# dcmlr/groundgrid

Measured on NVIDIA H100. Metric: Mpoints/sec segmented (64-beam scan), higher is better.
Workload: dtype f32/f64

## Files before the change

### groundgrid_b200/csrc/gg_capi.cu

```cuda
#include <cuda.h>
#include <cuda_runtime.h>

#include <cmath>
#include <cstdarg>
#include <cstdio>
#include <atomic>
#include <chrono>
#include <condition_variable>
#include <cstdlib>
#include <cstring>
#include <functional>
#include <initializer_list>
#include <mutex>
#include <string>
#include <thread>
#include <vector>

#include "gg_host.h"
#include "gg_internal.h"

namespace {

thread_local std::string g_last_error;

// ... 745 lines not shown
        v.visits = d_vs;
        v.levels = (int)ls.size() - 1;
        h->sched_levels = v.levels;
        h->sched_visits = (int)vs.size();
        for (size_t l = 0; l + 1 < ls.size(); ++l) h->sched_max = std::max(h->sched_max, ls[l + 1] - ls[l]);
        v.spiral_recs = nullptr;
        v.spiral_dist = 0;
        v.spiral_threads = h->sched_max <= 512 ? 512 : 1024;
        int dist = 2;
        if (const char* e = getenv("GG_SPIRAL_DIST")) dist = atoi(e);
        std::vector<uint32_t> rc;
        int max_recent = 0;
        if (dist >= 1 && dist <= 3 && h->sched_max <= 1024 && gg::build_spiral_records(n, v.k.res_sq, ls, vs, dist, rc, max_recent)) {
            uint32_t* d_rc = nullptr;
            GG_TRY(dev_alloc(h, &d_rc, rc.size() + 4));
            GG_CUDA_TRY(cudaMemcpy(d_rc, rc.data(), rc.size() * sizeof(uint32_t), cudaMemcpyHostToDevice));
            v.spiral_recs = reinterpret_cast<const uint4*>(d_rc);
            v.spiral_dist = dist;
        }
        std::memset(&v.skew, 0, sizeof(v.skew));
        int want_skew = 1;
        if (const char* e = getenv("GG_SPIRAL_SKEW")) want_skew = atoi(e);
        gg::SkewTables sk;
        if (want_skew) gg::build_spiral_skew(n, ls, vs, sk);
        int M = 32, phases = 1, M_thr = 32, phases_thr = 1;
        if (sk.ok) {
            const int kGap = 2 * 8 + 4;
            auto smallest_fitting = [&](int m0) {
                int m = m0;
                for (; m < sk.KP; m += 32) {
                    bool fits = true;
                    for (int sd = 0; sd < 4 && fits; ++sd)
                        for (int c0 = 0; c0 + m < sk.KP && fits; ++c0) {
                            const int a = sd * sk.KP + c0, b2 = a + m;
                            if (sk.lane_begin[a] < sk.lane_end[a] && sk.lane_begin[b2] < sk.lane_end[b2] &&
                                sk.lane_end[a] + kGap > sk.lane_begin[b2])
                                fits = false;
                        }
                    if (fits) break;
                }
                return std::min(m, sk.KP);
            };
            M = (4 * sk.KP + 64 <= 1024) ? sk.KP : smallest_fitting(32);
            phases = (sk.KP + M - 1) / M;
            int m0 = 0;
            if (const char* e = getenv("GG_SPIRAL_M")) m0 = atoi(e) / 32 * 32;
            M_thr = m0 <= 0 ? M : smallest_fitting(std::max(32, m0));
// ... 2 lines not shown
        }
        if (sk.ok) {
            const int irr_max = std::max(1, sk.max_irr_per_level);
            const int irr_words = ((irr_max * 22 + 3) / 4) * 4;
            std::vector<uint32_t> blocks((size_t)(sk.levels + 4) * irr_words, 0xffffffffu);
            for (int l = 0; l < sk.levels; ++l)
                for (int r = sk.irr_level_start[l]; r < sk.irr_level_start[l + 1]; ++r) {
                    const uint32_t* w = &sk.irr_recs[(size_t)r * 16];
                    const int vv = r - sk.irr_level_start[l];
                    uint32_t* blk = &blocks[(size_t)l * irr_words];
                    for (int q = 0; q < 9; ++q) {
                        blk[(vv * 9 + q) * 2] = w[1 + q];
                        blk[(vv * 9 + q) * 2 + 1] = 0xffffffffu;
                    }
                    const uint32_t ents[4] = {w[10] & 0xffffu, w[10] >> 16, w[11] & 0xffffu, w[11] >> 16};
                    for (uint32_t e : ents)
                        if (e != 0xffffu) blk[(vv * 9 + (e >> 12)) * 2 + 1] = e & 4095u;
                    uint32_t* hd = blk + irr_max * 18 + vv * 4;
                    hd[0] = w[0];
                    hd[1] = w[12];
                    hd[2] = w[13];
                    hd[3] = w[14];
                }
            auto upload_phases = [&](int m_, int phases_, const int** d_b, const int** d_e, const int** d_c) -> int {
                std::vector<int> ph_b((size_t)phases_ * 4 * m_, 0), ph_e((size_t)phases_ * 4 * m_, 0), ph_c((size_t)phases_ * 4 * m_, 0);
                for (int ph = 0; ph < phases_; ++ph)
                    for (int sd = 0; sd < 4; ++sd)
                        for (int m = 0; m < m_; ++m) {
                            const int col = ph * m_ + m;
                            if (col >= sk.KP) continue;
                            const size_t dst = ((size_t)ph * 4 + sd) * m_ + m;
                            ph_b[dst] = sk.lane_begin[sd * sk.KP + col];
                            ph_e[dst] = sk.lane_end[sd * sk.KP + col];
                            ph_c[dst] = sk.lane_cell0[sd * sk.KP + col];
                        }
                int *d_lb = nullptr, *d_le = nullptr, *d_lc = nullptr;
                int rc2;
                if ((rc2 = dev_alloc(h, &d_lb, ph_b.size())) || (rc2 = dev_alloc(h, &d_le, ph_e.size())) || (rc2 = dev_alloc(h, &d_lc, ph_c.size())))
                    return rc2;
                if (cudaMemcpy(d_lb, ph_b.data(), ph_b.size() * sizeof(int), cudaMemcpyHostToDevice) != cudaSuccess ||
                    cudaMemcpy(d_le, ph_e.data(), ph_e.size() * sizeof(int), cudaMemcpyHostToDevice) != cudaSuccess ||
                    cudaMemcpy(d_lc, ph_c.data(), ph_c.size() * sizeof(int), cudaMemcpyHostToDevice) != cudaSuccess)
                    return fail(GG_E_CUDA, "upload of the spiral phase tables failed");
                *d_b = d_lb;
                *d_e = d_le;
                *d_c = d_lc;
// ... 24 lines not shown
            int want_async = 0;
            if (const char* e = getenv("GG_SPIRAL_ASYNC")) want_async = atoi(e);
            auto upload_req = [&](int m_, const uint16_t** d_req) -> int {
                *d_req = nullptr;
                std::vector<uint16_t> rq;
                int n_agents = 0;
                if (!want_async || !gg::build_skew_sync(sk, m_, gg::SKEW_XCH_ASYNC, rq, n_agents)) return GG_OK;
                uint16_t* d = nullptr;
                int rc2;
                if ((rc2 = dev_alloc(h, &d, rq.size()))) return rc2;
                if (cudaMemcpy(d, rq.data(), rq.size() * sizeof(uint16_t), cudaMemcpyHostToDevice) != cudaSuccess)
                    return fail(GG_E_CUDA, "upload of the spiral synchronisation table failed");
                *d_req = d;
                return GG_OK;
            };
            v.skew.sync_sleep = 20;
            if (const char* e = getenv("GG_SPIRAL_SLEEP")) v.skew.sync_sleep = std::max(0, atoi(e));
            GG_TRY(upload_req(M, &v.skew.req));
            if (M_thr == M)
                v.skew.thr_req = v.skew.req;
            else
                GG_TRY(upload_req(M_thr, &v.skew.thr_req));
            v.skew.irr_blocks = reinterpret_cast<const uint4*>(d_irr);
            v.skew.irr_max = irr_max;
            v.skew.irr_chunks = irr_words / 4;
            v.skew.KP = sk.KP;
            v.skew.rows = sk.rows;
            v.skew.row0 = sk.row0;
            v.skew.lanes = sk.lanes;
            v.skew.levels = sk.levels;
            std::memcpy(v.skew.pattern, sk.pattern, sizeof(sk.pattern));
        }
    }

    if (const char* e = getenv("GG_LAUNCH_UNIT")) h->launch_unit = std::max(1, atoi(e));
    if (const char* e = getenv("GG_COPY_STREAMS")) h->n_copy_in = std::min(8, std::max(1, atoi(e)));
    if (const char* e = getenv("GG_MAIN_HELP")) h->main_help = atoi(e);
    if (const char* e = getenv("GG_RAW_GATE")) h->raw_gate = std::max(1, atoi(e));
    if (const char* e = getenv("GG_BUS_TARGET_MB")) h->bus_target = (size_t)std::max(0, atoi(e)) << 20;
    if (const char* e = getenv("GG_RAW_DEPTH")) h->raw_depth = std::min(8, std::max(1, atoi(e)));
    if (const char* e = getenv("GG_HOST_PACK")) {
        h->host_pack = atoi(e) ? 1 : 0;
        h->host_pack_mix = 0;
    }
    v.packed = nullptr;
    if (stream) {
// ... 1186 lines not shown
```

### groundgrid_b200/csrc/gg_host.cpp

```cpp
#include <immintrin.h>

#include <algorithm>
#include <cmath>
#include <cstdio>
#include <thread>
#include <cstdint>
#include <cpuid.h>
#include <cstdlib>
#include <cstring>
#include <vector>

#include <sched.h>

#include "gg_host.h"

namespace gg {

int cells_per_side(double dimension_m, float resolution) {
    return (int)std::round((float)dimension_m / resolution);
}

void build_expected_points(int n, std::vector<float>& table) {
    const float vertical_point_ang_dist = 0.00174532925 * 2;
    table.assign((size_t)n * n, 0.0f);
// ... 169 lines not shown
        }
        if (nr > 4) ok = false;
        max_recent = std::max(max_recent, nr);
        const float fx = (float)x - (float)c, fy = (float)y - (float)c;
        const bool far = ((double)fx * (double)fx + (double)fy * (double)fy) * res_sq > 12.0;
        recs[4 * (size_t)t + 0] = (uint32_t)x | ((uint32_t)y << 16);
        recs[4 * (size_t)t + 1] = r[0] | (r[1] << 16);
        recs[4 * (size_t)t + 2] = r[2] | (r[3] << 16);
        recs[4 * (size_t)t + 3] = (far ? 1u : 0u) | (seen[cell] ? 2u : 0u);
        last_writer[cell] = t;
        ++seen[cell];
    };
    for (int p = c - 1; p >= 1; --p) {
        const int side = (c - p) * 2;
        const int q = p + side;
        for (int pos = p; pos < q; ++pos) visit(p, pos);
        for (int pos = p; pos < q; ++pos) visit(pos, p);
        for (int pos = q; pos >= p; --pos) visit(q, pos);
        for (int pos = q; pos >= p; --pos) visit(pos, q);
    }
    return ok;
}

void build_spiral_skew(int n, const std::vector<int>& level_start, const std::vector<uint32_t>& visits, SkewTables& t) {
    t = SkewTables();
    t.n = n;
    const int c = n / 2 - 1;
    const int K = c - 1;
    t.K = K;
    t.levels = (int)level_start.size() - 1;
    if (K < 2) return;
    t.KP = ((K + 2 + 31) / 32) * 32;
    if (4 * t.KP > 4095) return;
    const size_t nv = visits.size();
    std::vector<std::vector<int>> cell_levels((size_t)n * n);
    for (int l = 0; l < t.levels; ++l)
        for (int v = level_start[l]; v < level_start[l + 1]; ++v) {
            const int x = visits[v] & 0xffff, y = visits[v] >> 16;
            cell_levels[x + (size_t)y * n].push_back(l);
        }
    struct Visit {
        int s, k, j, x, y, level;
    };
    std::vector<Visit> seq;
    seq.reserve(nv);
    std::vector<int> seen((size_t)n * n, 0);
    int max_level = 0;
    auto push = [&](int s, int k, int j, int x, int y) {
        const size_t cell = x + (size_t)y * n;
// ... 61 lines not shown
            const int* h = homes(v.x - 1 + q % 3, v.y - 1 + q / 3);
            for (int i = 0; i < 4 && h[i] >= 0; ++i) bump(v.s * 9 + q, h[i] - own);
        }
    }
    for (int i = 0; i < 36; ++i) {
        int best = 0, cnt = -1;
        for (auto& e : stat[i])
            if (e.second > cnt) {
                cnt = e.second;
                best = e.first;
            }
        if (cnt < 0) return;
        t.pattern[i] = best;
    }

    std::vector<int> last_level((size_t)n * n, -1000000), last_lane((size_t)n * n, -1);
    t.lane_begin.assign(t.lanes, 0);
    t.lane_end.assign(t.lanes, 0);
    t.lane_cell0.assign(t.lanes, 0);
    std::vector<int> reg_first(t.lanes, -1), reg_last(t.lanes, -1), reg_count(t.lanes, 0);
    struct Irr {
        int level;
        uint32_t w[16];
    };
    std::vector<Irr> irr;
    for (const Visit& v : seq) {
        const int lane = v.s * t.KP + (v.k + 1);
        const int own = slot(v.s, v.k, v.level);
        const size_t cell = v.x + (size_t)v.y * n;
        int nb[9];
        bool regular = true;
        uint32_t rec[4] = {0xffffu, 0xffffu, 0xffffu, 0xffffu};
        int nrec = 0;
        for (int q = 0; q < 9; ++q) {
            const int cx = v.x - 1 + q % 3, cy = v.y - 1 + q / 3;
            const int* h = homes(cx, cy);
            if (h[0] < 0) return;
            const int want = own + t.pattern[v.s * 9 + q];
            bool match = false;
            for (int i = 0; i < 4 && h[i] >= 0; ++i) match |= (h[i] == want);
            nb[q] = match ? want : h[0];
            if (!match) regular = false;
            const size_t ncell = cx + (size_t)cy * n;
            const int back = v.level - last_level[ncell];
            if (back < 1) return;
            if (back == 1) {
                if (!(q == t.prev_q[v.s] && last_lane[ncell] == lane)) regular = false;
                if (nrec < 4) rec[nrec] = ((uint32_t)q << 12) | (uint32_t)last_lane[ncell];
                ++nrec;
            }
        }
        if (nrec > 4) return;
        if (nrec != 1) regular = false;
        const int* hown = homes(v.x, v.y);
        int mirror = -1;
        if (hown[1] >= 0) {
            regular = false;
            mirror = (hown[0] == own) ? hown[1] : hown[0];
            if (hown[2] >= 0) return;
        }
        {
            SkewTables::Access a;
            a.level = v.level;
            a.lane = lane;
            a.own = own;
            a.mirror = mirror;
            a.cell = (int)cell;
            a.regular = regular;
            for (int q = 0; q < 9; ++q) {
                a.nb[q] = nb[q];
                a.recent_lane[q] = -1;
            }
            for (int e = 0; e < 4; ++e)
                if (rec[e] != 0xffffu) a.recent_lane[rec[e] >> 12] = (int)(rec[e] & 4095u);
            t.acc.push_back(a);
        }
        if (regular) {
            ++t.n_regular;
            if (reg_first[lane] < 0) {
                reg_first[lane] = v.level;
                t.lane_cell0[lane] = (int)cell;
            }
            if (reg_last[lane] >= 0 && v.level != reg_last[lane] + 1) return;
            reg_last[lane] = v.level;
            ++reg_count[lane];
        } else {
            ++t.n_irregular;
            Irr r;
            r.level = v.level;
            std::memset(r.w, 0, sizeof(r.w));
            r.w[0] = (uint32_t)own;
            for (int q = 0; q < 9; ++q) r.w[1 + q] = (uint32_t)nb[q];
            r.w[10] = rec[0] | (rec[1] << 16);
            r.w[11] = rec[2] | (rec[3] << 16);
            r.w[12] = (uint32_t)mirror;
            r.w[13] = (uint32_t)lane;
            r.w[14] = (uint32_t)cell;
            irr.push_back(r);
        }
        last_level[cell] = v.level;
        last_lane[cell] = lane;
    }
    for (int l = 0; l < t.lanes; ++l)
        if (reg_first[l] >= 0) {
            t.lane_begin[l] = reg_first[l];
            t.lane_end[l] = reg_last[l] + 1;
            if (t.lane_end[l] - t.lane_begin[l] != reg_count[l]) return;
        }
    t.irr_level_start.assign((size_t)t.levels + 1, 0);
    for (const Irr& r : irr) ++t.irr_level_start[(size_t)r.level + 1];
    for (int l = 0; l < t.levels; ++l) {
        t.max_irr_per_level = std::max(t.max_irr_per_level, t.irr_level_start[(size_t)l + 1]);
        t.irr_level_start[(size_t)l + 1] += t.irr_level_start[l];
    }
    if (t.max_irr_per_level > 32) return;
    t.irr_recs.assign(irr.size() * 16, 0u);
    std::vector<int> cur(t.irr_level_start.begin(), t.irr_level_start.end() - 1);
    for (const Irr& r : irr) std::memcpy(&t.irr_recs[(size_t)cur[r.level]++ * 16], r.w, sizeof(r.w));
    t.ok = true;
}

bool build_skew_sync(const SkewTables& t, int M, int xch_depth, std::vector<uint16_t>& req, int& n_agents) {
    req.clear();
    n_agents = 0;
    if (!t.ok || M < 32 || (M % 32) != 0 || xch_depth < 2 || (xch_depth & (xch_depth - 1))) return false;
    const int lane_agents = 4 * M / 32;
    if (lane_agents + 1 > 32 || t.levels >= 65535) return false;
    n_agents = lane_agents + 1;
    const int IRR = lane_agents, L = t.levels;
    req.assign((size_t)n_agents * L * 32, 0);
    bool ok = true;
    auto agent_of = [&](const SkewTables::Access& a) {
        if (!a.regular) return IRR;
        const int side = a.lane / t.KP, col = a.lane % t.KP;
        return (side * M + col % M) / 32;
    };
    auto need = [&](int a, int lvl, int b, int done) {
        if (a == b || b < 0) return;
        if (lvl < 0) lvl = 0;
        if (done + 1 > lvl) {
            if (getenv("GG_SYNC_DEBUG")) fprintf(stderr, "sync: agent %d level %d needs agent %d done %d\n", a, lvl, b, done);
// ... 274 lines not shown
    if (ok && req && req_cap >= (int)r.size()) std::memcpy(req, r.data(), r.size() * sizeof(uint16_t));
    return ok ? 1 : 0;
}

int gg_host_spiral_skew(int n, int* header, int* pattern, int* lane_begin, int* lane_end, int* cell_home, int* irr_level_start,
                        uint32_t* irr_recs, int irr_cap_words) {
    std::vector<int> ls;
    std::vector<uint32_t> vs;
    gg::build_spiral_schedule(n, ls, vs);
    gg::SkewTables t;
    gg::build_spiral_skew(n, ls, vs, t);
    const int h[10] = {t.ok ? 1 : 0, t.K, t.KP, t.rows, t.levels, t.row0, t.lanes, (int)t.n_irregular, t.max_irr_per_level, (int)t.n_regular};
    std::memcpy(header, h, sizeof(h));
    if (!t.ok) return 0;
    if (pattern) std::memcpy(pattern, t.pattern, sizeof(t.pattern));
    if (lane_begin) std::memcpy(lane_begin, t.lane_begin.data(), t.lane_begin.size() * sizeof(int));
    if (lane_end) std::memcpy(lane_end, t.lane_end.data(), t.lane_end.size() * sizeof(int));
    if (cell_home) std::memcpy(cell_home, t.cell_home.data(), t.cell_home.size() * sizeof(int));
    if (irr_level_start) std::memcpy(irr_level_start, t.irr_level_start.data(), t.irr_level_start.size() * sizeof(int));
    if (irr_recs && irr_cap_words >= (int)t.irr_recs.size()) std::memcpy(irr_recs, t.irr_recs.data(), t.irr_recs.size() * sizeof(uint32_t));
    return 1;
}

int gg_host_move_map(double res, double* pos_xy, double nx, double ny, int* shift_ij) {
    gg::move_map(res, pos_xy[0], pos_xy[1], nx, ny, shift_ij[0], shift_ij[1]);
    return (shift_ij[0] != 0 || shift_ij[1] != 0) ? 1 : 0;
}

int gg_host_geometry_constants(double dimension_m, float resolution, unsigned flags, double* out) {
    gg::Const k;
    gg::derive_geometry(dimension_m, resolution, flags, k);
    const double v[9] = {(double)k.N, (double)k.N2, (double)k.full_layers, (double)k.res_f, k.res, k.rres, k.len, k.half, k.res_sq};
    std::memcpy(out, v, sizeof(v));
    return 0;
}

int gg_host_config_constants(const gg_config* cfg, double* out) {
    gg::CfgConst k;
    gg::derive_config(*cfg, k);
    const double v[16] = {(double)k.max_ring, (double)k.pc_var_thresh_f, k.min_outlier_conf, k.outlier_tol, k.gp_thresh, k.df_sq, k.mdf_sq,
                          k.mdf10_sq, k.psc_sq, k.occ_factor, k.occ_factor2, k.dec_factor, k.lab_fac, k.lab_thres, k.lab_obs,
                          (double)k.decay_floor_ok};
    std::memcpy(out, v, sizeof(v));
    return 0;
}

// ... 32 lines not shown
```

### groundgrid_b200/csrc/gg_host.h

```cpp
#pragma once
#include <cstdint>
#include <vector>

#include "gg_internal.h"

namespace gg {
int cells_per_side(double dimension_m, float resolution);
void build_expected_points(int n, std::vector<float>& table);
void derive_geometry(double dimension_m, float resolution, unsigned flags, Const& k);
void derive_config(const gg_config& c, CfgConst& k);

class ConfigRegistry {
  public:
    void reset(int n_slots, const CfgConst& k);
    int assign(int slot, const CfgConst& k, bool* build);
    void invalidate(int id) { vars_[id].k.reserved = 1; }
    int variant_of(int slot) const { return slot_var_[slot]; }
    const CfgConst& constants(int id) const { return vars_[id].k; }
    int refs(int id) const { return vars_[id].refs; }
    int live() const;
    int ids() const { return (int)vars_.size(); }

  private:
    struct Variant {
// ... 2 lines not shown
    };
    std::vector<Variant> vars_;
    std::vector<int> slot_var_;
};
void move_map(double res, double& px, double& py, double nx, double ny, int& shift_i, int& shift_j);
void build_spiral_schedule(int n, std::vector<int>& level_start, std::vector<uint32_t>& visits);
void pack_cloud_range(const gg_point* src, size_t n, unsigned char* dst, size_t i0, size_t i1, bool cached = false);
int usable_cpus();

struct SkewTables {
    bool ok = false;
    int n = 0, K = 0, KP = 0, rows = 0, levels = 0, row0 = 8;
    int lanes = 0;
    size_t slots = 0;
    int pattern[36] = {0};
    int prev_q[4] = {1, 3, 7, 5};
    std::vector<int> lane_begin, lane_end;
    std::vector<int> lane_cell0;
    std::vector<int> cell_home;
    std::vector<int> irr_level_start;
    std::vector<uint32_t> irr_recs;
    int max_irr_per_level = 0;
    size_t n_regular = 0, n_irregular = 0;
    struct Access {
        int level, lane;
        int own, mirror, cell;
        int nb[9];
        int recent_lane[9];
        bool regular;
    };
    std::vector<Access> acc;
};
bool build_skew_sync(const SkewTables& t, int M, int xch_depth, std::vector<uint16_t>& req, int& n_agents);
void build_spiral_skew(int n, const std::vector<int>& level_start, const std::vector<uint32_t>& visits, SkewTables& t);
bool build_spiral_records(int n, double res_sq, const std::vector<int>& level_start, const std::vector<uint32_t>& visits,
                          int dist, std::vector<uint32_t>& recs, int& max_recent);
}

extern "C" {
int gg_host_cells_per_side(double dimension_m, float resolution);
int gg_host_expected_points(double dimension_m, float resolution, float* dst);
int gg_host_spiral_schedule(int n, int* level_start, int level_cap, uint32_t* visits, int visit_cap, int* n_levels, int* n_visits);
int gg_host_spiral_records(int n, float resolution, int dist, uint32_t* recs, int rec_cap_words, int* max_recent);
int gg_host_move_map(double res, double* pos_xy, double nx, double ny, int* shift_ij);
int gg_host_geometry_constants(double dimension_m, float resolution, unsigned flags, double* out);
int gg_host_config_constants(const gg_config* cfg, double* out);
int gg_host_config_registry(int n_slots, int n_ops, const int* op_slot, const gg_config* op_cfg, int* out);
int gg_host_pack_cloud(const gg_point* src, size_t n, unsigned char* dst);
int gg_host_pack_cloud_cached(const gg_point* src, size_t n, unsigned char* dst);
int gg_host_packer_selftest(int threads, int n_jobs, size_t n_points, int ring_slots, int rounds, int lag);
int gg_host_spiral_skew_sync(int n, int M, int xch_depth, uint16_t* req, int req_cap, int* n_agents);
int gg_host_spiral_skew(int n, int* header, int* pattern, int* lane_begin, int* lane_end, int* cell_home, int* irr_level_start, uint32_t* irr_recs, int irr_cap_words);
}
```

### groundgrid_b200/csrc/gg_internal.h

```cpp
#pragma once
#include <cuda.h>
#include <cuda_runtime.h>
#include <stdint.h>

#include "groundgrid_b200.h"

namespace gg {

enum Layer : int {
    L_GROUND = 0,
    L_GROUNDPATCH = 1,
    L_OBSTACLES = 2,
    L_VARIANCE = 3,
    L_MINH = 4,
    L_COUNT = 5,
    L_MAXH = 6,
    L_GCAND = 7,
    L_PLANEDIST = 8,
    L_M2 = 9,
    L_MEAN = 10,
    L_RAW = 11,
    L_NUM = 12,
    L_NUM_LIVE = 6,
};
// ... 34 lines not shown
    CfgConst cfg;
    const float4* detect_tab;
    double px, py;
    double t20, t21, t22, t23;
    float ox, oy, oz;
    float base_z_f;
    int n_points;
    int shift_i, shift_j;
    int slot;
    const gg_point* src;
    const float* packed;
};

struct OutDest {
    uint8_t* labels;
    uint32_t* index;
    gg_point* cloud;
    int* count;
    unsigned select;
    int reserved;
};

constexpr int SKEW_XCH_ASYNC = 4;
struct SkewView {
    float2* sk;
    float* sd;
    size_t slots;
    const int* cell_home;
    const int* ph_begin;
    const int* ph_end;
    const int* ph_cell0;
    int M, phases;
    const int* thr_ph_begin;
    const int* thr_ph_end;
    const int* thr_ph_cell0;
    int thr_M, thr_phases;
    const uint16_t* req;
    const uint16_t* thr_req;
    int sync_sleep;
    const uint4* irr_blocks;
    int irr_max, irr_chunks;
    int KP, rows, row0, lanes, levels;
    int pattern[36];
};

struct View {
    Const k;
    float* layers;
    int n_layers;
    const float* expected;
    gg_point* points;
    unsigned char* packed;
    uint2* zw;
    uint32_t* runj;
    float* zsorted;
    uint2* rundir;
    float* dist;
    uint32_t* code;
    uint8_t* labels;
    unsigned long long* cnt64;
    int* raw_i;
    int* cellstart;
    int4* worklist;
    int* wl_count;
    int* cell_agg;
    int cell_tiles;
// ... 68 lines not shown
```

### groundgrid_b200/csrc/gg_kernels.cu

```cuda
#include <cuda.h>

#include <cfloat>
#include <cstddef>
#include <cstdio>

#include "gg_internal.h"

namespace gg {
constexpr int GRID_STRIDE_BLOCKS = 132;

__device__ __forceinline__ int trunc_index(double v) {
    if (!(v == v)) return 1000000000;
    if (v > 1.0e9) return 1000000000;
    if (v < -1.0e9) return -1000000000;
    return __double2int_rz(v);
}

__device__ __forceinline__ int trunc_quotient(double a, double res, double rres) {
    const double q = __dmul_rn(a, rres);
    const double f = __dsub_rn(q, rint(q));
    if (fabs(q) < 1.0e6 && fabs(f) > 1.0e-6) return __double2int_rz(q);
    return trunc_index(__ddiv_rn(a, res));
}

// ... 1225 lines not shown
}

constexpr int SKEW_IRR_THREADS = 64;
constexpr int SKEW_RING = 16;
constexpr int SKEW_STAGE_LEAD = 10;

__device__ __forceinline__ void prefetch_l2(const void* p) { asm volatile("prefetch.global.L2 [%0];" ::"l"(p)); }
__device__ __forceinline__ void prefetch_l1(const void* p) { asm volatile("prefetch.global.L1 [%0];" ::"l"(p)); }

__device__ __forceinline__ void skew_publish(int* s_prog, int agent, int completed, int lane) {
    __syncwarp();
    if (lane == 0) asm volatile("st.release.cta.shared.u32 [%0], %1;" ::"r"(smem_u32(s_prog + agent)), "r"(completed) : "memory");
}
__device__ __forceinline__ void skew_wait(const int* s_prog, int need, int lane, int sleep_ns) {
    const uint32_t addr = smem_u32(s_prog + lane);
    for (;;) {
        int p;
        asm volatile("ld.acquire.cta.shared.u32 %0, [%1];" : "=r"(p) : "r"(addr) : "memory");
        if (__all_sync(0xffffffffu, p >= need)) break;
        if (sleep_ns) __nanosleep(sleep_ns);
    }
}

template <int SIDE, bool ASYNC>
__device__ __forceinline__ void skew_lane_thread(const View& v, const SlotParams& sp, float2* s_xch, int* s_prog) {
    const SkewView& w = v.skew;
    constexpr int XM = (ASYNC ? SKEW_XCH_ASYNC : 2) - 1;
    const int lane_id = threadIdx.x & 31;
    const int agent = threadIdx.x >> 5;
    const uint16_t* __restrict__ req = ASYNC ? w.req + (size_t)agent * w.levels * 32 + lane_id : nullptr;
    int need_nxt = ASYNC ? (int)__ldg(req) : 0;
    constexpr int PQ = SIDE == 0 ? 1 : (SIDE == 1 ? 3 : (SIDE == 2 ? 7 : 5));
    constexpr int PF_FAR = 8, PF_NEAR = 2;
    const int L = w.levels, KP = w.KP, lanes = w.lanes, M = w.M;
    const int m = threadIdx.x - SIDE * M;
    float2* __restrict__ SK = w.sk + (size_t)sp.slot * w.slots;
    const float* __restrict__ SD = w.sd + (size_t)sp.slot * w.slots;
    float* __restrict__ Gn = v.layer(sp.slot, L_GROUND);
    float* __restrict__ Cn = v.layer(sp.slot, L_GROUNDPATCH);
    const int cstep = SIDE == 0 ? v.k.N : (SIDE == 1 ? 1 : (SIDE == 2 ? -v.k.N : -1));
    int off[9];
#pragma unroll
    for (int q = 0; q < 9; ++q) off[q] = w.pattern[SIDE * 9 + q];
    int off_new = off[0];
#pragma unroll
    for (int q = 1; q < 9; ++q) off_new = max(off_new, off[q]);

    int ph = -1, lb = 0, le = 0, base0 = 0, cell0 = 0, xid = 0;
    int w_first = 0, w_last = 0;
    auto next_phase = [&]() {
        ++ph;
        const size_t e = ((size_t)ph * 4 + SIDE) * M + m;
        const int col = ph * M + m;
        lb = w.ph_begin[e];
        le = w.ph_end[e];
        base0 = (SIDE * w.rows + w.row0) * KP + col;
        cell0 = w.ph_cell0[e] - lb * cstep;
        xid = SIDE * KP + col;
    };
    auto warp_window = [&]() {
        w_first = lb < le ? lb - PF_FAR : 0x7fffffff;
        w_last = lb < le ? le : -1;
#pragma unroll
        for (int d = 16; d >= 1; d >>= 1) {
            w_first = min(w_first, __shfl_xor_sync(0xffffffffu, w_first, d));
            w_last = max(w_last, __shfl_xor_sync(0xffffffffu, w_last, d));
        }
        w_first = max(w_first, 0) & ~1;
    };
    next_phase();
    warp_window();

    float2 A[9], B[9];
    float dA = -1.0f, dB = -1.0f;
#pragma unroll
    for (int q = 0; q < 9; ++q) A[q] = B[q] = make_float2(0.f, 0.f);
    if (lb == 0 && le > 0) {
#pragma unroll
        for (int q = 0; q < 9; ++q) A[q] = SK[base0 + off[q]];
        dA = SD[base0];
    }
#define GG_LANE_LEVEL(l_, CUR, CURD, NXT, NXTD)                                                      \
    {                                                                                               \
        const int l__ = (l_);                                                                       \
        if (ASYNC) {                                                                                \
            const int need__ = need_nxt;                                                            \
            if (l__ + 1 < L) need_nxt = (int)__ldg(req + (size_t)(l__ + 1) * 32);                   \
            skew_wait(s_prog, need__, lane_id, w.sync_sleep);                                                     \
        }                                                                                           \
        if (l__ + PF_FAR >= lb && l__ + PF_FAR < le) {                                              \
            prefetch_l2(SK + (base0 + (l__ + PF_FAR) * KP + off_new));                              \
            prefetch_l2(SD + (base0 + (l__ + PF_FAR) * KP));                                        \
        }                                                                                           \
        if (l__ + PF_NEAR >= lb && l__ + PF_NEAR < le) {                                            \
            prefetch_l1(SK + (base0 + (l__ + PF_NEAR) * KP + off_new));                             \
            prefetch_l1(SD + (base0 + (l__ + PF_NEAR) * KP));                                       \
        }                                                                                           \
        if (l__ + 1 >= lb && l__ + 1 < le) {                                                        \
            const float2* p__ = SK + (base0 + (l__ + 1) * KP);                                      \
            _Pragma("unroll") for (int q = 0; q < 9; ++q) NXT[q] = p__[off[q]];                    \
            NXTD = SD[base0 + (l__ + 1) * KP];                                                      \
        }                                                                                           \
        if (l__ >= lb && l__ < le) {                                                                \
            CUR[PQ] = s_xch[((l__ - 1) & XM) * lanes + xid];                                        \
            const float2 r__ = spiral_visit(CUR, CURD);                                             \
            s_xch[(l__ & XM) * lanes + xid] = r__;                                                  \
            SK[base0 + l__ * KP] = r__;                                                             \
            Gn[cell0 + l__ * cstep] = r__.x;                                                        \
            if (CURD >= 0.0f) Cn[cell0 + l__ * cstep] = r__.y;                                      \
        }                                                                                           \
        if (ASYNC)                                                                                  \
            skew_publish(s_prog, agent, l__ + 1, lane_id);                                          \
        else                                                                                        \
            __syncthreads();                                                                        \
    }
    for (int l = 0; l < L; l += 2) {
        if (w.phases > 1) {
            bool moved = false;
            while (ph + 1 < w.phases && l >= le) {
                next_phase();
                moved = true;
            }
            if (__any_sync(0xffffffffu, moved)) warp_window();
        }
        if (l < w_first || l >= w_last) {
            if (ASYNC) {
                skew_publish(s_prog, agent, min(l + 2, L), lane_id);
                if (l + 2 < L) need_nxt = (int)__ldg(req + (size_t)(l + 2) * 32);
            } else {
                __syncthreads();
                if (l + 1 < L) __syncthreads();
            }
            continue;
        }
        GG_LANE_LEVEL(l, A, dA, B, dB)
        if (l + 1 < L) GG_LANE_LEVEL(l + 1, B, dB, A, dA)
    }
#undef GG_LANE_LEVEL
}

__device__ __forceinline__ void skew_named_barrier() { asm volatile("bar.sync 1, %0;" ::"n"(SKEW_IRR_THREADS) : "memory"); }

template <bool ASYNC>
__device__ __forceinline__ void skew_irregular_thread(const View& v, const SlotParams& sp, float2* s_xch, uint4* s_ring, float2* s_nb, float* s_dd, int* s_prog) {
    const SkewView& w = v.skew;
    const int ti = threadIdx.x - 4 * w.M;
    constexpr int XM = (ASYNC ? SKEW_XCH_ASYNC : 2) - 1;
    const int lane_id = threadIdx.x & 31;
    const int agent = 4 * w.M / 32;
    const uint16_t* __restrict__ req = ASYNC ? w.req + (size_t)agent * w.levels * 32 + lane_id : nullptr;
    int need_nxt = ASYNC ? (int)__ldg(req) : 0;
    const int L = w.levels, lanes = w.lanes;
    const int chunks = w.irr_chunks, irr_max = w.irr_max;
    float2* __restrict__ SK = w.sk + (size_t)sp.slot * w.slots;
    const float* __restrict__ SD = w.sd + (size_t)sp.slot * w.slots;
    const uint4* __restrict__ blocks = w.irr_blocks;
    float* __restrict__ Gn = v.layer(sp.slot, L_GROUND);
    float* __restrict__ Cn = v.layer(sp.slot, L_GROUNDPATCH);
    if (ti == 0) {
        const int cidx = v.k.N / 2 - 1;
        Cn[cidx + cidx * v.k.N] = 1.0f;
        Gn[cidx + cidx * v.k.N] = sp.base_z_f;
    }
    const uint32_t* ring_w = reinterpret_cast<const uint32_t*>(s_ring);
    const int ring_words = chunks * 4;
    const bool stager = ti < chunks;
    const bool gatherer = ti < irr_max * 9;
    const bool visitor = ti < irr_max;

    if (stager) {
        for (int b = 0; b < SKEW_STAGE_LEAD; ++b) s_ring[b * chunks + ti] = blocks[(size_t)min(b, L + 3) * chunks + ti];
    }
    uint4 stage = stager ? blocks[(size_t)min(SKEW_STAGE_LEAD, L + 3) * chunks + ti] : make_uint4(0, 0, 0, 0);
    skew_named_barrier();
    float2 val = make_float2(0.f, 0.f);
    float dval = -1.0f;
    uint32_t info = 0xffffffffu;
    bool have = false;
    if (gatherer) {
        const uint32_t slot = ring_w[0 * ring_words + ti * 2], rl = ring_w[0 * ring_words + ti * 2 + 1];
        have = slot != 0xffffffffu;
        if (have) {
            val = SK[slot];
            info = rl;
            if (ti % 9 == 4) dval = SD[slot];
        }
    }
    for (int l = 0; l < L; ++l) {
        if (ASYNC) {
            const int need = need_nxt;
            if (l + 1 < L) need_nxt = (int)__ldg(req + (size_t)(l + 1) * 32);
            skew_wait(s_prog, need, lane_id, w.sync_sleep);
        }
        if (stager) {
            s_ring[((l + SKEW_STAGE_LEAD) % SKEW_RING) * chunks + ti] = stage;
            stage = blocks[(size_t)min(l + SKEW_STAGE_LEAD + 1, L + 3) * chunks + ti];
        }
        if (gatherer) {
            if (have) {
                if (info != 0xffffffffu) val = s_xch[((l - 1) & XM) * lanes + (int)info];
                s_nb[ti] = val;
                if (ti % 9 == 4) s_dd[ti / 9] = dval;
            }
            const uint32_t far_slot = ring_w[((l + SKEW_STAGE_LEAD - 2) % SKEW_RING) * ring_words + ti * 2];
            if (far_slot != 0xffffffffu) {
                prefetch_l2(SK + far_slot);
                if (ti % 9 == 4) prefetch_l2(SD + far_slot);
            }
            const uint32_t near_slot = ring_w[((l + 3) % SKEW_RING) * ring_words + ti * 2];
            if (near_slot != 0xffffffffu) {
                prefetch_l1(SK + near_slot);
                if (ti % 9 == 4) prefetch_l1(SD + near_slot);
            }
            const uint32_t* e = ring_w + ((l + 1) % SKEW_RING) * ring_words + ti * 2;
            const uint32_t slot = e[0];
            have = (l + 1 < L) && slot != 0xffffffffu;
            if (have) {
                val = SK[slot];
                info = e[1];
                if (ti % 9 == 4) dval = SD[slot];
            }
        }
        skew_named_barrier();
        if (visitor) {
            const uint32_t* hd = ring_w + (l % SKEW_RING) * ring_words + irr_max * 18 + ti * 4;
            const uint32_t own = hd[0];
            if (own != 0xffffffffu) {
                float2 nb[9];
#pragma unroll
                for (int q = 0; q < 9; ++q) nb[q] = s_nb[ti * 9 + q];
                const float2 r = spiral_visit(nb, s_dd[ti]);
                const int mirror = (int)hd[1];
                s_xch[(l & XM) * lanes + (int)hd[2]] = r;
                SK[own] = r;
                if (mirror >= 0) SK[mirror] = r;
                Gn[hd[3]] = r.x;
                if (s_dd[ti] >= 0.0f) Cn[hd[3]] = r.y;
            }
        }
        if (ASYNC) {
            skew_named_barrier();
            if (ti == 0) asm volatile("st.release.cta.shared.u32 [%0], %1;" ::"r"(smem_u32(s_prog + agent)), "r"(l + 1) : "memory");
        } else {
            __syncthreads();
        }
    }
}

template <int MAXT, int MIN_CTAS = 1, bool ASYNC = false>
__global__ void __launch_bounds__(MAXT, MIN_CTAS) k_spiral_skew(View v, const SlotParams* __restrict__ batch) {
    extern __shared__ __align__(16) unsigned char s_raw[];
    const SkewView& w = v.skew;
    uint4* s_ring = reinterpret_cast<uint4*>(s_raw);
    float2* s_xch = reinterpret_cast<float2*>(s_ring + SKEW_RING * w.irr_chunks);
    float2* s_nb = s_xch + (ASYNC ? SKEW_XCH_ASYNC : 2) * w.lanes;
    float* s_dd = reinterpret_cast<float*>(s_nb + w.irr_max * 9);
    int* s_prog = reinterpret_cast<int*>(s_dd + w.irr_max);
    const SlotParams& sp = batch[blockIdx.x];
    const int tid = threadIdx.x;
    if (ASYNC) {
        if (tid < 32) s_prog[tid] = tid <= 4 * w.M / 32 ? 0 : 0x7fffffff;
        __syncthreads();
    }
    if (tid < 4 * w.M) {
        const int side = tid / w.M;
        if (side == 0)
            skew_lane_thread<0, ASYNC>(v, sp, s_xch, s_prog);
        else if (side == 1)
            skew_lane_thread<1, ASYNC>(v, sp, s_xch, s_prog);
        else if (side == 2)
            skew_lane_thread<2, ASYNC>(v, sp, s_xch, s_prog);
        else
            skew_lane_thread<3, ASYNC>(v, sp, s_xch, s_prog);
    } else {
        skew_irregular_thread<ASYNC>(v, sp, s_xch, s_ring, s_nb, s_dd, s_prog);
    }
}

constexpr int LABEL_ILP = 4;

__global__ void __launch_bounds__(256) k_label(View v, const SlotParams* __restrict__ batch) {
    const SlotParams& sp = batch[blockIdx.y];
    const Const& k = v.k;
    const size_t base = (size_t)sp.slot * v.pcap;
    const int i0 = blockIdx.x * (256 * LABEL_ILP) + threadIdx.x;
    const int n = sp.n_points;
    if (i0 >= n) return;
    const float* L0 = v.layer(sp.slot, 0);
    const float* G = L0 + L_GROUND * k.N2;
    const float* V = L0 + L_VARIANCE * k.N2;
    float* OBS = v.layer(sp.slot, L_OBSTACLES);

    uint32_t code[LABEL_ILP];
    float dist[LABEL_ILP], z[LABEL_ILP], gh[LABEL_ILP], var[LABEL_ILP];
#pragma unroll
    for (int u = 0; u < LABEL_ILP; ++u) {
        const int i = i0 + u * 256;
        const bool in = i < n;
        code[u] = in ? v.code[base + i] : (PC_ABSENT << 24);
// ... 418 lines not shown
        else
            GG_LAUNCH(K_DETECT, k_detect_tma<4><<<tgrid, dim3(DT_X, DT_Y), 0, st>>>(v, batch, *layer_map));
    } else if (detect_occ >= 5)
        GG_LAUNCH(K_DETECT, k_detect_ldg<5><<<dgrid, dim3(DT_X, DT_Y), 0, st>>>(v, batch));
    else
        GG_LAUNCH(K_DETECT, k_detect_ldg<4><<<dgrid, dim3(DT_X, DT_Y), 0, st>>>(v, batch));
    ++launches;
    if (after_detect) cudaEventRecord(after_detect, st);
    if (stop_after == 2) return launches;

    if (v.skew.sk) {
        static const int share_min = getenv("GG_SPIRAL_SHARE_MIN") ? atoi(getenv("GG_SPIRAL_SHARE_MIN")) : 9;
        View vs = v;
        if (count >= share_min) {
            vs.skew.M = v.skew.thr_M;
            vs.skew.phases = v.skew.thr_phases;
            vs.skew.ph_begin = v.skew.thr_ph_begin;
            vs.skew.ph_end = v.skew.thr_ph_end;
            vs.skew.ph_cell0 = v.skew.thr_ph_cell0;
            vs.skew.req = v.skew.thr_req;
        }
        const bool async = vs.skew.req != nullptr;
        const int threads = 4 * vs.skew.M + SKEW_IRR_THREADS;
        const size_t shm = (size_t)SKEW_RING * v.skew.irr_chunks * sizeof(uint4) + (size_t)(async ? SKEW_XCH_ASYNC : 2) * v.skew.lanes * sizeof(float2) +
                           (size_t)v.skew.irr_max * 9 * sizeof(float2) + (size_t)v.skew.irr_max * sizeof(float) + 32 * sizeof(int) + 16;
#define GG_SKEW_LAUNCH(T, C)                                                                                                     \
    {                                                                                                                            \
        if (shm > 48 * 1024) {                                            \
            cudaFuncSetAttribute(k_spiral_skew<T, C, false>, cudaFuncAttributeMaxDynamicSharedMemorySize, (int)shm);             \
            cudaFuncSetAttribute(k_spiral_skew<T, C, true>, cudaFuncAttributeMaxDynamicSharedMemorySize, (int)shm);              \
        }                                                                                                                        \
        if (async)                                                                                                               \
            GG_LAUNCH(K_SPIRAL, (k_spiral_skew<T, C, true><<<count, threads, shm, st>>>(vs, batch)));                            \
        else                                                                                                                     \
            GG_LAUNCH(K_SPIRAL, (k_spiral_skew<T, C, false><<<count, threads, shm, st>>>(vs, batch)));                           \
    }
        if (threads <= 320)
            GG_SKEW_LAUNCH(320, 3)
        else if (threads <= 448)
            GG_SKEW_LAUNCH(448, 2)
        else if (threads <= 768)
            GG_SKEW_LAUNCH(768, 1)
        else
            GG_SKEW_LAUNCH(1024, 1)
#undef GG_SKEW_LAUNCH
    } else if (v.spiral_recs) {
        const size_t shm = (size_t)((v.levels + 4) & ~3) * sizeof(int) + (size_t)(v.spiral_dist + 1) * v.spiral_threads * sizeof(float2);
#define GG_SPIRAL_CASE(T, D)                                                                      \
    if (v.spiral_threads == T && v.spiral_dist == D) {                                            \
        if (shm > 48 * 1024) cudaFuncSetAttribute(k_spiral_pipe<T, D>, cudaFuncAttributeMaxDynamicSharedMemorySize, (int)shm); \
        GG_LAUNCH(K_SPIRAL, k_spiral_pipe<T, D><<<count, T, shm, st>>>(v, batch));                \
    }
        GG_SPIRAL_CASE(512, 1)
        GG_SPIRAL_CASE(512, 2)
        GG_SPIRAL_CASE(512, 3)
        GG_SPIRAL_CASE(1024, 1)
        GG_SPIRAL_CASE(1024, 2)
        GG_SPIRAL_CASE(1024, 3)
#undef GG_SPIRAL_CASE
    } else {
// ... 151 lines not shown
```

Before: 4940.

## Keep spiral neighbour values in a shared-memory level window instead of global copies

Adds a windowed variant of the skewed spiral kernel that keeps the last eight levels of results in shared memory and reads neighbour values from that ring instead of from global SK copies. The host checks that no lane overwrites a ring slot before its consumer reads it, and falls back to the old path otherwise. This removes global stores of mirror/own copies and their reloads. The cost is more shared memory per block, a 64-register cap, and extra host table building.

After: 5050 (median of 6 runs). 1.02x the previous value.

```diff
diff --git a/groundgrid_b200/csrc/gg_capi.cu b/groundgrid_b200/csrc/gg_capi.cu
--- a/groundgrid_b200/csrc/gg_capi.cu
+++ b/groundgrid_b200/csrc/gg_capi.cu
@@ -791,7 +791,18 @@
         int want_skew = 1;
         if (const char* e = getenv("GG_SPIRAL_SKEW")) want_skew = atoi(e);
         gg::SkewTables sk;
-        if (want_skew) gg::build_spiral_skew(n, ls, vs, sk);
+        int want_window = 1;
+        if (const char* e = getenv("GG_SPIRAL_WINDOW")) want_window = atoi(e);
+        if (want_skew) {
+            gg::build_spiral_skew(n, ls, vs, sk, want_window != 0);
+            if (sk.window) {
+                int smem_optin = 0;
+                cudaDeviceGetAttribute(&smem_optin, cudaDevAttrMaxSharedMemoryPerBlockOptin, h->device);
+                const size_t win_bytes = (size_t)gg::SKEW_WIN_ROWS * sk.lanes * sizeof(float2) + 16 * 1024;
+                if (!sk.ok || ((sk.win_bad >> (gg::SKEW_WIN_ROWS - 1)) & 1) || win_bytes > (size_t)smem_optin)
+                    gg::build_spiral_skew(n, ls, vs, sk);
+            }
+        }
         int M = 32, phases = 1, M_thr = 32, phases_thr = 1;
         if (sk.ok) {
             const int kGap = 2 * 8 + 4;
@@ -840,6 +851,18 @@
                     hd[2] = w[13];
                     hd[3] = w[14];
                 }
+            std::vector<uint32_t> win_blocks;
+            if (sk.window) {
+                win_blocks = blocks;
+                for (int l = 0; l < sk.levels; ++l)
+                    for (int r = sk.irr_level_start[l]; r < sk.irr_level_start[l + 1]; ++r)
+                        for (int q = 0; q < 9; ++q) {
+                            const uint32_t e = sk.irr_win[(size_t)r * 9 + q];
+                            const int row = (l - (int)(e >> 16)) & (gg::SKEW_WIN_ROWS - 1);
+                            win_blocks[(size_t)l * irr_words + ((r - sk.irr_level_start[l]) * 9 + q) * 2 + 1] =
+                                e == 0xffffffffu ? e : (uint32_t)(row * sk.lanes + (int)(e & 0xffffu));
+                        }
+            }
             auto upload_phases = [&](int m_, int phases_, const int** d_b, const int** d_e, const int** d_c) -> int {
                 std::vector<int> ph_b((size_t)phases_ * 4 * m_, 0), ph_e((size_t)phases_ * 4 * m_, 0), ph_c((size_t)phases_ * 4 * m_, 0);
                 for (int ph = 0; ph < phases_; ++ph)
@@ -910,6 +933,13 @@
             else
                 GG_TRY(upload_req(M_thr, &v.skew.thr_req));
             v.skew.irr_blocks = reinterpret_cast<const uint4*>(d_irr);
+            if (sk.window) {
+                uint32_t* d_win = nullptr;
+                GG_TRY(dev_alloc(h, &d_win, win_blocks.size() + 16));
+                GG_CUDA_TRY(cudaMemcpy(d_win, win_blocks.data(), win_blocks.size() * sizeof(uint32_t), cudaMemcpyHostToDevice));
+                v.skew.win_blocks = reinterpret_cast<const uint4*>(d_win);
+                v.skew.win = 1;
+            }
             v.skew.irr_max = irr_max;
             v.skew.irr_chunks = irr_words / 4;
             v.skew.KP = sk.KP;
diff --git a/groundgrid_b200/csrc/gg_host.cpp b/groundgrid_b200/csrc/gg_host.cpp
--- a/groundgrid_b200/csrc/gg_host.cpp
+++ b/groundgrid_b200/csrc/gg_host.cpp
@@ -215,9 +215,10 @@
     return ok;
 }
 
-void build_spiral_skew(int n, const std::vector<int>& level_start, const std::vector<uint32_t>& visits, SkewTables& t) {
+void build_spiral_skew(int n, const std::vector<int>& level_start, const std::vector<uint32_t>& visits, SkewTables& t, bool window) {
     t = SkewTables();
     t.n = n;
+    t.window = window;
     const int c = n / 2 - 1;
     const int K = c - 1;
     t.K = K;
@@ -325,6 +326,7 @@
     struct Irr {
         int level;
         uint32_t w[16];
+        uint32_t win[9];
     };
     std::vector<Irr> irr;
     for (const Visit& v : seq) {
@@ -335,6 +337,7 @@
         bool regular = true;
         uint32_t rec[4] = {0xffffu, 0xffffu, 0xffffu, 0xffffu};
         int nrec = 0;
+        int lastl[9], lastn[9];
         for (int q = 0; q < 9; ++q) {
             const int cx = v.x - 1 + q % 3, cy = v.y - 1 + q / 3;
             const int* h = homes(cx, cy);
@@ -352,6 +355,13 @@
                 if (nrec < 4) rec[nrec] = ((uint32_t)q << 12) | (uint32_t)last_lane[ncell];
                 ++nrec;
             }
+            const bool visited = last_level[ncell] >= 0;
+            lastl[q] = visited ? last_level[ncell] : -1;
+            lastn[q] = visited ? last_lane[ncell] : -1;
+            if (window) {
+                const int wb = skew_win_back(v.s, q);
+                if (visited ? (back != wb || last_lane[ncell] != lane - (q == t.prev_q[v.s] ? 0 : 1)) : wb != 0) regular = false;
+            }
         }
         if (nrec > 4) return;
         if (nrec != 1) regular = false;
@@ -373,6 +383,8 @@
             for (int q = 0; q < 9; ++q) {
                 a.nb[q] = nb[q];
                 a.recent_lane[q] = -1;
+                a.last_level[q] = lastl[q];
+                a.last_lane[q] = lastn[q];
             }
             for (int e = 0; e < 4; ++e)
                 if (rec[e] != 0xffffu) a.recent_lane[rec[e] >> 12] = (int)(rec[e] & 4095u);
@@ -399,6 +411,8 @@
             r.w[12] = (uint32_t)mirror;
             r.w[13] = (uint32_t)lane;
             r.w[14] = (uint32_t)cell;
+            for (int q = 0; q < 9; ++q)
+                r.win[q] = lastl[q] >= 0 ? ((uint32_t)(v.level - lastl[q]) << 16) | (uint32_t)lastn[q] : 0xffffffffu;
             irr.push_back(r);
         }
         last_level[cell] = v.level;
@@ -419,7 +433,33 @@
     if (t.max_irr_per_level > 32) return;
     t.irr_recs.assign(irr.size() * 16, 0u);
     std::vector<int> cur(t.irr_level_start.begin(), t.irr_level_start.end() - 1);
-    for (const Irr& r : irr) std::memcpy(&t.irr_recs[(size_t)cur[r.level]++ * 16], r.w, sizeof(r.w));
+    if (window) t.irr_win.assign(irr.size() * 9, 0u);
+    for (const Irr& r : irr) {
+        const size_t i = (size_t)cur[r.level]++;
+        std::memcpy(&t.irr_recs[i * 16], r.w, sizeof(r.w));
+        if (window) std::memcpy(&t.irr_win[i * 9], r.win, sizeof(r.win));
+    }
+    if (window) {
+        std::vector<std::vector<char>> writes((size_t)t.lanes, std::vector<char>((size_t)t.levels, 0));
+        for (const SkewTables::Access& a : t.acc) writes[(size_t)a.lane][(size_t)a.level] = 1;
+        constexpr int DMAX = 64;
+        std::vector<char> bad(DMAX + 1, 0);
+        for (const SkewTables::Access& a : t.acc)
+            for (int q = 0; q < 9; ++q) {
+                if (a.last_level[q] < 0) continue;
+                const std::vector<char>& wl = writes[(size_t)a.last_lane[q]];
+                for (int lw = a.last_level[q] + 1; lw <= a.level; ++lw)
+                    if (wl[(size_t)lw])
+                        for (int d = 1; d <= DMAX; ++d)
+                            if ((lw - a.last_level[q]) % d == 0) bad[d] = 1;
+            }
+        for (int d = DMAX; d >= 1; --d)
+            if (bad[d])
+                t.win_bad |= 1ull << (d - 1);
+            else
+                t.win_depth = d;
+        if (!t.win_depth) return;
+    }
     t.ok = true;
 }
 
@@ -740,6 +780,32 @@
     return 1;
 }
 
+int gg_host_spiral_window(int n, int* header, int* win_back, int* lane_begin, int* lane_end, int* lane_cell0, int* cell_home, int* irr_level_start,
+                          uint32_t* irr_recs, uint32_t* irr_win, int irr_cap) {
+    std::vector<int> ls;
+    std::vector<uint32_t> vs;
+    gg::build_spiral_schedule(n, ls, vs);
+    gg::SkewTables t0, t;
+    gg::build_spiral_skew(n, ls, vs, t0);
+    gg::build_spiral_skew(n, ls, vs, t, true);
+    const int h[14] = {t.ok ? 1 : 0, t.K, t.KP, t.rows, t.levels, t.row0, t.lanes, (int)t.n_irregular, t.max_irr_per_level, (int)t.n_regular,
+                       t.win_depth, (t.win_bad >> (gg::SKEW_WIN_ROWS - 1)) & 1 ? 0 : 1, gg::SKEW_WIN_ROWS, (int)t0.n_regular};
+    std::memcpy(header, h, sizeof(h));
+    if (!t.ok) return 0;
+    if (win_back)
+        for (int i = 0; i < 36; ++i) win_back[i] = gg::skew_win_back(i / 9, i % 9);
+    if (lane_begin) std::memcpy(lane_begin, t.lane_begin.data(), t.lane_begin.size() * sizeof(int));
+    if (lane_end) std::memcpy(lane_end, t.lane_end.data(), t.lane_end.size() * sizeof(int));
+    if (lane_cell0) std::memcpy(lane_cell0, t.lane_cell0.data(), t.lane_cell0.size() * sizeof(int));
+    if (cell_home) std::memcpy(cell_home, t.cell_home.data(), t.cell_home.size() * sizeof(int));
+    if (irr_level_start) std::memcpy(irr_level_start, t.irr_level_start.data(), t.irr_level_start.size() * sizeof(int));
+    if (irr_cap >= (int)t.n_irregular) {
+        if (irr_recs) std::memcpy(irr_recs, t.irr_recs.data(), t.irr_recs.size() * sizeof(uint32_t));
+        if (irr_win) std::memcpy(irr_win, t.irr_win.data(), t.irr_win.size() * sizeof(uint32_t));
+    }
+    return 1;
+}
+
 int gg_host_move_map(double res, double* pos_xy, double nx, double ny, int* shift_ij) {
     gg::move_map(res, pos_xy[0], pos_xy[1], nx, ny, shift_ij[0], shift_ij[1]);
     return (shift_ij[0] != 0 || shift_ij[1] != 0) ? 1 : 0;
diff --git a/groundgrid_b200/csrc/gg_host.h b/groundgrid_b200/csrc/gg_host.h
--- a/groundgrid_b200/csrc/gg_host.h
+++ b/groundgrid_b200/csrc/gg_host.h
@@ -48,17 +48,22 @@
     std::vector<uint32_t> irr_recs;
     int max_irr_per_level = 0;
     size_t n_regular = 0, n_irregular = 0;
+    bool window = false;
+    int win_depth = 0;
+    uint64_t win_bad = 0;
+    std::vector<uint32_t> irr_win;
     struct Access {
         int level, lane;
         int own, mirror, cell;
         int nb[9];
         int recent_lane[9];
+        int last_level[9], last_lane[9];
         bool regular;
     };
     std::vector<Access> acc;
 };
 bool build_skew_sync(const SkewTables& t, int M, int xch_depth, std::vector<uint16_t>& req, int& n_agents);
-void build_spiral_skew(int n, const std::vector<int>& level_start, const std::vector<uint32_t>& visits, SkewTables& t);
+void build_spiral_skew(int n, const std::vector<int>& level_start, const std::vector<uint32_t>& visits, SkewTables& t, bool window = false);
 bool build_spiral_records(int n, double res_sq, const std::vector<int>& level_start, const std::vector<uint32_t>& visits,
                           int dist, std::vector<uint32_t>& recs, int& max_recent);
 }
@@ -77,4 +82,6 @@
 int gg_host_packer_selftest(int threads, int n_jobs, size_t n_points, int ring_slots, int rounds, int lag);
 int gg_host_spiral_skew_sync(int n, int M, int xch_depth, uint16_t* req, int req_cap, int* n_agents);
 int gg_host_spiral_skew(int n, int* header, int* pattern, int* lane_begin, int* lane_end, int* cell_home, int* irr_level_start, uint32_t* irr_recs, int irr_cap_words);
+int gg_host_spiral_window(int n, int* header, int* win_back, int* lane_begin, int* lane_end, int* lane_cell0, int* cell_home, int* irr_level_start,
+                          uint32_t* irr_recs, uint32_t* irr_win, int irr_cap);
 }
diff --git a/groundgrid_b200/csrc/gg_internal.h b/groundgrid_b200/csrc/gg_internal.h
--- a/groundgrid_b200/csrc/gg_internal.h
+++ b/groundgrid_b200/csrc/gg_internal.h
@@ -80,6 +80,14 @@
 };
 
 constexpr int SKEW_XCH_ASYNC = 4;
+constexpr int SKEW_WIN_ROWS = 8;
+__host__ __device__ constexpr int skew_win_back(int s, int q) {
+    constexpr int t[36] = {0, 1, 5, 0, 0, 4, 0, 0, 3,
+                           0, 0, 0, 1, 0, 0, 5, 4, 3,
+                           3, 0, 0, 4, 0, 0, 5, 1, 0,
+                           3, 4, 5, 0, 0, 1, 0, 0, 0};
+    return t[s * 9 + q];
+}
 struct SkewView {
     float2* sk;
     float* sd;
@@ -100,6 +108,8 @@
     int irr_max, irr_chunks;
     int KP, rows, row0, lanes, levels;
     int pattern[36];
+    const uint4* win_blocks;
+    int win;
 };
 
 struct View {
diff --git a/groundgrid_b200/csrc/gg_kernels.cu b/groundgrid_b200/csrc/gg_kernels.cu
--- a/groundgrid_b200/csrc/gg_kernels.cu
+++ b/groundgrid_b200/csrc/gg_kernels.cu
@@ -1271,10 +1271,10 @@
     }
 }
 
-template <int SIDE, bool ASYNC>
+template <int SIDE, bool ASYNC, bool WINDOW = false>
 __device__ __forceinline__ void skew_lane_thread(const View& v, const SlotParams& sp, float2* s_xch, int* s_prog) {
     const SkewView& w = v.skew;
-    constexpr int XM = (ASYNC ? SKEW_XCH_ASYNC : 2) - 1;
+    constexpr int XM = (WINDOW ? SKEW_WIN_ROWS : (ASYNC ? SKEW_XCH_ASYNC : 2)) - 1;
     const int lane_id = threadIdx.x & 31;
     const int agent = threadIdx.x >> 5;
     const uint16_t* __restrict__ req = ASYNC ? w.req + (size_t)agent * w.levels * 32 + lane_id : nullptr;
@@ -1294,6 +1294,7 @@
     int off_new = off[0];
 #pragma unroll
     for (int q = 1; q < 9; ++q) off_new = max(off_new, off[q]);
+    auto from_copy = [](int q) { return !WINDOW || skew_win_back(SIDE, q) == 0; };
 
     int ph = -1, lb = 0, le = 0, base0 = 0, cell0 = 0, xid = 0;
     int w_first = 0, w_last = 0;
@@ -1326,7 +1327,8 @@
     for (int q = 0; q < 9; ++q) A[q] = B[q] = make_float2(0.f, 0.f);
     if (lb == 0 && le > 0) {
 #pragma unroll
-        for (int q = 0; q < 9; ++q) A[q] = SK[base0 + off[q]];
+        for (int q = 0; q < 9; ++q)
+            if (from_copy(q)) A[q] = SK[base0 + off[q]];
         dA = SD[base0];
     }
 #define GG_LANE_LEVEL(l_, CUR, CURD, NXT, NXTD)                                                      \
@@ -1347,14 +1349,19 @@
         }                                                                                           \
         if (l__ + 1 >= lb && l__ + 1 < le) {                                                        \
             const float2* p__ = SK + (base0 + (l__ + 1) * KP);                                      \
-            _Pragma("unroll") for (int q = 0; q < 9; ++q) NXT[q] = p__[off[q]];                    \
+            _Pragma("unroll") for (int q = 0; q < 9; ++q) if (from_copy(q)) NXT[q] = p__[off[q]];  \
             NXTD = SD[base0 + (l__ + 1) * KP];                                                      \
         }                                                                                           \
         if (l__ >= lb && l__ < le) {                                                                \
-            CUR[PQ] = s_xch[((l__ - 1) & XM) * lanes + xid];                                        \
+            if (WINDOW) {                                                                           \
+                _Pragma("unroll") for (int q = 0; q < 9; ++q) if (!from_copy(q))                    \
+                    CUR[q] = s_xch[((l__ - skew_win_back(SIDE, q)) & XM) * lanes + xid - (q == PQ ? 0 : 1)]; \
+            } else {                                                                                \
+                CUR[PQ] = s_xch[((l__ - 1) & XM) * lanes + xid];                                    \
+            }                                                                                       \
             const float2 r__ = spiral_visit(CUR, CURD);                                             \
             s_xch[(l__ & XM) * lanes + xid] = r__;                                                  \
-            SK[base0 + l__ * KP] = r__;                                                             \
+            if (!WINDOW) SK[base0 + l__ * KP] = r__;                                                \
             Gn[cell0 + l__ * cstep] = r__.x;                                                        \
             if (CURD >= 0.0f) Cn[cell0 + l__ * cstep] = r__.y;                                      \
         }                                                                                           \
@@ -1390,11 +1397,11 @@
 
 __device__ __forceinline__ void skew_named_barrier() { asm volatile("bar.sync 1, %0;" ::"n"(SKEW_IRR_THREADS) : "memory"); }
 
-template <bool ASYNC>
+template <bool ASYNC, bool WINDOW = false>
 __device__ __forceinline__ void skew_irregular_thread(const View& v, const SlotParams& sp, float2* s_xch, uint4* s_ring, float2* s_nb, float* s_dd, int* s_prog) {
     const SkewView& w = v.skew;
     const int ti = threadIdx.x - 4 * w.M;
-    constexpr int XM = (ASYNC ? SKEW_XCH_ASYNC : 2) - 1;
+    constexpr int XM = (WINDOW ? SKEW_WIN_ROWS : (ASYNC ? SKEW_XCH_ASYNC : 2)) - 1;
     const int lane_id = threadIdx.x & 31;
     const int agent = 4 * w.M / 32;
     const uint16_t* __restrict__ req = ASYNC ? w.req + (size_t)agent * w.levels * 32 + lane_id : nullptr;
@@ -1403,7 +1410,7 @@
     const int chunks = w.irr_chunks, irr_max = w.irr_max;
     float2* __restrict__ SK = w.sk + (size_t)sp.slot * w.slots;
     const float* __restrict__ SD = w.sd + (size_t)sp.slot * w.slots;
-    const uint4* __restrict__ blocks = w.irr_blocks;
+    const uint4* __restrict__ blocks = WINDOW ? w.win_blocks : w.irr_blocks;
     float* __restrict__ Gn = v.layer(sp.slot, L_GROUND);
     float* __restrict__ Cn = v.layer(sp.slot, L_GROUNDPATCH);
     if (ti == 0) {
@@ -1430,7 +1437,7 @@
         const uint32_t slot = ring_w[0 * ring_words + ti * 2], rl = ring_w[0 * ring_words + ti * 2 + 1];
         have = slot != 0xffffffffu;
         if (have) {
-            val = SK[slot];
+            if (!WINDOW || rl == 0xffffffffu) val = SK[slot];
             info = rl;
             if (ti % 9 == 4) dval = SD[slot];
         }
@@ -1447,7 +1454,7 @@
         }
         if (gatherer) {
             if (have) {
-                if (info != 0xffffffffu) val = s_xch[((l - 1) & XM) * lanes + (int)info];
+                if (info != 0xffffffffu) val = WINDOW ? s_xch[info] : s_xch[((l - 1) & XM) * lanes + (int)info];
                 s_nb[ti] = val;
                 if (ti % 9 == 4) s_dd[ti / 9] = dval;
             }
@@ -1465,8 +1472,13 @@
             const uint32_t slot = e[0];
             have = (l + 1 < L) && slot != 0xffffffffu;
             if (have) {
-                val = SK[slot];
-                info = e[1];
+                if (WINDOW) {
+                    info = e[1];
+                    if (info == 0xffffffffu) val = SK[slot];
+                } else {
+                    val = SK[slot];
+                    info = e[1];
+                }
                 if (ti % 9 == 4) dval = SD[slot];
             }
         }
@@ -1481,8 +1493,10 @@
                 const float2 r = spiral_visit(nb, s_dd[ti]);
                 const int mirror = (int)hd[1];
                 s_xch[(l & XM) * lanes + (int)hd[2]] = r;
-                SK[own] = r;
-                if (mirror >= 0) SK[mirror] = r;
+                if (!WINDOW) {
+                    SK[own] = r;
+                    if (mirror >= 0) SK[mirror] = r;
+                }
                 Gn[hd[3]] = r.x;
                 if (s_dd[ti] >= 0.0f) Cn[hd[3]] = r.y;
             }
@@ -1496,13 +1510,14 @@
     }
 }
 
-template <int MAXT, int MIN_CTAS = 1, bool ASYNC = false>
-__global__ void __launch_bounds__(MAXT, MIN_CTAS) k_spiral_skew(View v, const SlotParams* __restrict__ batch) {
+template <bool ASYNC, bool WINDOW>
+__device__ __forceinline__ void spiral_skew_cta(const View& v, const SlotParams* __restrict__ batch) {
+    static_assert(!(ASYNC && WINDOW), "the level window is a variant of the barrier kernel");
     extern __shared__ __align__(16) unsigned char s_raw[];
     const SkewView& w = v.skew;
     uint4* s_ring = reinterpret_cast<uint4*>(s_raw);
     float2* s_xch = reinterpret_cast<float2*>(s_ring + SKEW_RING * w.irr_chunks);
-    float2* s_nb = s_xch + (ASYNC ? SKEW_XCH_ASYNC : 2) * w.lanes;
+    float2* s_nb = s_xch + (WINDOW ? SKEW_WIN_ROWS : (ASYNC ? SKEW_XCH_ASYNC : 2)) * w.lanes;
     float* s_dd = reinterpret_cast<float*>(s_nb + w.irr_max * 9);
     int* s_prog = reinterpret_cast<int*>(s_dd + w.irr_max);
     const SlotParams& sp = batch[blockIdx.x];
@@ -1514,16 +1529,25 @@
     if (tid < 4 * w.M) {
         const int side = tid / w.M;
         if (side == 0)
-            skew_lane_thread<0, ASYNC>(v, sp, s_xch, s_prog);
+            skew_lane_thread<0, ASYNC, WINDOW>(v, sp, s_xch, s_prog);
         else if (side == 1)
-            skew_lane_thread<1, ASYNC>(v, sp, s_xch, s_prog);
+            skew_lane_thread<1, ASYNC, WINDOW>(v, sp, s_xch, s_prog);
         else if (side == 2)
-            skew_lane_thread<2, ASYNC>(v, sp, s_xch, s_prog);
+            skew_lane_thread<2, ASYNC, WINDOW>(v, sp, s_xch, s_prog);
         else
-            skew_lane_thread<3, ASYNC>(v, sp, s_xch, s_prog);
+            skew_lane_thread<3, ASYNC, WINDOW>(v, sp, s_xch, s_prog);
     } else {
-        skew_irregular_thread<ASYNC>(v, sp, s_xch, s_ring, s_nb, s_dd, s_prog);
-    }
+        skew_irregular_thread<ASYNC, WINDOW>(v, sp, s_xch, s_ring, s_nb, s_dd, s_prog);
+    }
+}
+
+template <int MAXT, int MIN_CTAS = 1, bool ASYNC = false>
+__global__ void __launch_bounds__(MAXT, MIN_CTAS) k_spiral_skew(View v, const SlotParams* __restrict__ batch) {
+    spiral_skew_cta<ASYNC, false>(v, batch);
+}
+
+__global__ void __maxnreg__(64) k_spiral_skew_win(View v, const SlotParams* __restrict__ batch) {
+    spiral_skew_cta<false, true>(v, batch);
 }
 
 constexpr int LABEL_ILP = 4;
@@ -1988,7 +2012,9 @@
         }
         const bool async = vs.skew.req != nullptr;
         const int threads = 4 * vs.skew.M + SKEW_IRR_THREADS;
-        const size_t shm = (size_t)SKEW_RING * v.skew.irr_chunks * sizeof(uint4) + (size_t)(async ? SKEW_XCH_ASYNC : 2) * v.skew.lanes * sizeof(float2) +
+        const bool window = v.skew.win && !async && threads > 448;
+        const size_t shm = (size_t)SKEW_RING * v.skew.irr_chunks * sizeof(uint4) +
+                           (size_t)(window ? SKEW_WIN_ROWS : (async ? SKEW_XCH_ASYNC : 2)) * v.skew.lanes * sizeof(float2) +
                            (size_t)v.skew.irr_max * 9 * sizeof(float2) + (size_t)v.skew.irr_max * sizeof(float) + 32 * sizeof(int) + 16;
 #define GG_SKEW_LAUNCH(T, C)                                                                                                     \
     {                                                                                                                            \
@@ -2001,7 +2027,10 @@
         else                                                                                                                     \
             GG_LAUNCH(K_SPIRAL, (k_spiral_skew<T, C, false><<<count, threads, shm, st>>>(vs, batch)));                           \
     }
-        if (threads <= 320)
+        if (window) {
+            if (shm > 48 * 1024) cudaFuncSetAttribute(k_spiral_skew_win, cudaFuncAttributeMaxDynamicSharedMemorySize, (int)shm);
+            GG_LAUNCH(K_SPIRAL, (k_spiral_skew_win<<<count, threads, shm, st>>>(vs, batch)));
+        } else if (threads <= 320)
             GG_SKEW_LAUNCH(320, 3)
         else if (threads <= 448)
             GG_SKEW_LAUNCH(448, 2)
```
